# ziniuwan/maed

Hardware: AMD Instinct MI355X
Metric: video-clips/sec (BxT frames) train step (higher is better)
Workload: dtype bf16

## Files before the change

include/maed_hip.h:

```cpp
#ifndef MAED_HIP_H
#define MAED_HIP_H

#include <stddef.h>
#include <stdint.h>

#ifdef __cplusplus
extern "C" {
#endif

typedef enum { MAED_F32 = 0, MAED_BF16 = 1,
               MAED_F32X3 = 2, MAED_F32X6 = 3,
               MAED_F32X1 = 4 } maed_dtype;

typedef enum {
    MAED_OK = 0,
    MAED_ERR_ARG = -1,
    MAED_ERR_SHAPE = -2,
    MAED_ERR_ALIGN = -3,
    MAED_ERR_LAUNCH = -4,
    MAED_ERR_UNSUPPORTED = -5
} maed_status;

typedef enum {
    MAED_EPI_STORE = 0,
// ... 25 lines not shown
    MAED_OPT_ABLATE = 3,
    MAED_OPT_GN_BWD_ONEPASS = 4,
    MAED_OPT_F32_BWD_X1 = 5,
    MAED_OPT_ST_FUSED = 6,
    MAED_OPT_CONV3X3_ROWS_WGS = 7,
    MAED_OPT_STEM_WGRAD_WGS = 8,
    MAED_OPT_LBS_FRAMES = 9,
    MAED_OPT_TN_DMA = 10,
    MAED_OPT_X3_PLANES = 11,
    MAED_OPT_X3_PLANES_LN = 12,
    MAED_OPT_SK = 13,
    MAED_OPT_SK_GRID = 14,
    MAED_OPT_TN_SK = 15,
    MAED_OPT_CONV3X3_NARROW_WGS = 16,
    MAED_OPT_CONV3X3_FRAME = 17,
    MAED_OPT_COUNT
} maed_option;
int maed_init(int device);
int maed_device_faults(void);
int maed_device_faults_clear(void);
int maed_set_option(int key, int value);
int maed_get_option(int key);

int maed_layernorm_fwd(const float* x, int64_t x_row_stride, const float* gamma, const float* beta,
                       void* y, int dtype, float* mean, float* rstd,
                       int64_t rows, int C, float eps, void* stream);
int maed_layernorm_bwd(const void* dy, int dtype, const float* x, int64_t x_row_stride,
                       const float* gamma, const float* mean, const float* rstd,
                       const float* dres_in, float* dx_out, void* dx_twin, float* dgamma, float* dbeta,
                       int64_t rows, int C, void* stream);

int maed_gemm_nt(const void* A, int64_t lda, const void* B, int64_t ldb,
                 int64_t M, int64_t N, int64_t K, int dtype, int epilogue,
                 const float* bias, void* out, int64_t ldo, void* out2,
                 const void* aux, int64_t ldaux, int splitk, int impl, void* stream);

int maed_gemm_nt_planes(const void* a_hi, const void* a_lo, int64_t lda, const void* b_hi, const void* b_lo, int64_t ldb, int64_t M, int64_t N, int64_t K,
                        int epilogue, const float* bias, void* out, int64_t ldo, void* out2_bf16, const void* aux, int64_t ldaux, void* out_hi, void* out_lo,
                        int variant, void* stream);
int maed_split_planes(const float* x, void* hi, void* lo, int64_t n, void* stream);

int maed_gemm_tn_wgrad(const void* Y, int64_t ldy, const void* X, int64_t ldx, int64_t M, int N, int K,
                       float* dW, int64_t ldw, float* dbias, int dtype, void* stream);

int maed_transpose_cast(const void* in, int in_dtype, int64_t ldi, int64_t M, int64_t N,
                        void* out_t, int64_t ldt, void* out_c, int64_t ldc, float* colsum,
                        int dtype, void* stream);

int maed_attn_spatial_fwd(const void* qkv, void* o, float* lse, int F, int P, int H, float scale,
                          int dtype, int impl, void* stream);
int maed_attn_spatial_bwd(const void* qkv, const void* o, const void* d_o, const float* lse,
                          void* dqkv, int accumulate, int F, int P, int H, float scale,
                          int dtype, int impl, void* stream);

int maed_attn_temporal_fwd(const void* qkv, void* o, float* lse, int F, int P, int H, int T,
                           float scale, int dtype, void* stream);
int maed_attn_temporal_bwd(const void* qkv, const void* o, const void* d_o, const float* lse,
                           void* dqkv, int accumulate, int F, int P, int H, int T, float scale,
// ... 208 lines not shown
```

maed_amd/_lib.py:

```python
import ctypes as C
import os

HERE = os.path.dirname(os.path.abspath(__file__))
LIB_PATH = os.environ.get("MAED_HIP_LIB") or os.path.join(HERE, "libmaed_hip.so")

F32, BF16 = 0, 1
F32X3, F32X6, F32X1 = 2, 3, 4
EPI_STORE, EPI_GELU, EPI_RESID_F32, EPI_MUL_DGELU, EPI_ATOMIC_F32, EPI_STORE_F32, EPI_TANH, EPI_ADD = range(8)
IMPL_AUTO, IMPL_VALU, IMPL_MFMA = 0, 1, 2
IMPL_MFMA_256 = 6
IMPL_MFMA_LONG = 5
IMPL_MFMA_SK = 10
IMPL_X3, IMPL_X6, IMPL_X1 = 7, 8, 9
(OPT_F32_MATMUL, OPT_SIDE_STREAM, OPT_TN_TARGET_WGS, OPT_ABLATE, OPT_GN_BWD_ONEPASS, OPT_F32_BWD_X1, OPT_ST_FUSED, OPT_CONV3X3_ROWS_WGS, OPT_STEM_WGRAD_WGS,
 OPT_LBS_FRAMES, OPT_TN_DMA, OPT_X3_PLANES, OPT_X3_PLANES_LN, OPT_SK, OPT_SK_GRID, OPT_TN_SK, OPT_CONV3X3_NARROW_WGS, OPT_CONV3X3_FRAME) = range(18)

vp, i64, i32, f32 = C.c_void_p, C.c_int64, C.c_int, C.c_float


class GnAffineItem(C.Structure):
    _fields_ = [("ab", C.c_void_p), ("dgamma", C.c_void_p), ("dbeta", C.c_void_p), ("N", C.c_int), ("C", C.c_int)]


class BlockDims(C.Structure):
    _fields_ = [("F", i32), ("P", i32), ("C", i32), ("H", i32), ("T", i32), ("hidden", i32),
                ("dtype", i32), ("impl", i32), ("eps", f32)]


_PARAM_FIELDS = ["ln1_g", "ln1_b", "ln2_g", "ln2_b", "w_qkv", "w_ts", "w_proj", "w_fc1", "w_fc2",
                 "b_qkv", "b_ts", "b_proj", "b_fc1", "b_fc2", "wt_qkv", "wt_ts", "wt_proj", "wt_fc1", "wt_fc2"]
_GRAD_FIELDS = _PARAM_FIELDS[:14]


class BlockParams(C.Structure):
    _fields_ = [(n, vp) for n in _PARAM_FIELDS]

# ... 15 lines not shown


KTD_W_ANC = 3420

SIGNATURES = {
    "maed_last_error": (C.c_char_p, []),
    "maed_version": (i32, []),
    "maed_init": (i32, [i32]),
    "maed_device_faults": (i32, []),
    "maed_device_faults_clear": (i32, []),
    "maed_set_option": (i32, [i32, i32]),
    "maed_get_option": (i32, [i32]),
    "maed_layernorm_fwd": (i32, [vp, i64, vp, vp, vp, i32, vp, vp, i64, i32, f32, vp]),
    "maed_layernorm_bwd": (i32, [vp, i32, vp, i64, vp, vp, vp, vp, vp, vp, vp, vp, i64, i32, vp]),
    "maed_gemm_tn_wgrad": (i32, [vp, i64, vp, i64, i64, i32, i32, vp, i64, vp, i32, vp]),
    "maed_gemm_nt": (i32, [vp, i64, vp, i64, i64, i64, i64, i32, i32, vp, vp, i64, vp, vp, i64, i32, i32, vp]),
    "maed_transpose_cast": (i32, [vp, i32, i64, i64, i64, vp, i64, vp, i64, vp, i32, vp]),
    "maed_attn_spatial_fwd": (i32, [vp, vp, vp, i32, i32, i32, f32, i32, i32, vp]),
    "maed_attn_spatial_bwd": (i32, [vp, vp, vp, vp, vp, i32, i32, i32, i32, f32, i32, i32, vp]),
    "maed_attn_temporal_fwd": (i32, [vp, vp, vp, i32, i32, i32, i32, f32, i32, vp]),
    "maed_attn_temporal_bwd": (i32, [vp, vp, vp, vp, vp, i32, i32, i32, i32, i32, f32, i32, vp]),
    "maed_st_colmean": (i32, [vp, vp, vp, vp, i32, i32, i32, i32, vp]),
    "maed_st_mix_fwd": (i32, [vp, vp, vp, vp, i32, i32, i32, i32, vp]),
    "maed_st_mix_bwd_reduce": (i32, [vp, vp, vp, vp, vp, vp, i32, i32, i32, i32, vp]),
    "maed_st_mix_bwd_apply": (i32, [vp, vp, vp, vp, vp, i32, i32, i32, i32, vp]),
    "maed_st_fused_supported": (i32, [i32, i32, i32]),
    "maed_st_fused_fwd": (i32, [vp, vp, vp, vp, vp, vp, vp, vp, vp, i32, i32, i32, i32, vp]),
    "maed_st_fused_bwd": (i32, [vp, vp, vp, vp, vp, vp, vp, vp, vp, vp, i32, i32, i32, i32, vp]),
    "maed_embed_add_fwd": (i32, [vp, i32, vp, vp, vp, vp, i32, i32, i32, i32, vp]),
    "maed_embed_add_bwd": (i32, [vp, vp, i32, vp, vp, i32, i32, i32, i32, vp]),
# ... 109 lines not shown
    OPT_TN_TARGET_WGS: int(os.environ.get("MAED_TN_TARGET_WGS", "0")),
    OPT_ABLATE: int(os.environ.get("MAED_GEMM_ABLATE", "0")),
    OPT_F32_BWD_X1: int(os.environ.get("MAED_F32_BWD", "") == "bf16x1"),
    OPT_ST_FUSED: int(os.environ.get("MAED_ST_FUSED", "1")),
    OPT_GN_BWD_ONEPASS: int(os.environ.get("MAED_GN_BWD_ONEPASS", "1")),
    OPT_CONV3X3_ROWS_WGS: 0 if os.environ.get("MAED_CONV3X3_WGRAD_ROWS", "1") == "0" else int(os.environ.get("MAED_CONV3X3_ROWS_WGS", "256")),
    OPT_STEM_WGRAD_WGS: int(os.environ.get("MAED_STEM_WGS", "512")),
    OPT_LBS_FRAMES: int(os.environ.get("MAED_LBS_FB", "0")),
    OPT_TN_DMA: int(os.environ.get("MAED_TN_DMA", "1")),
    OPT_X3_PLANES: int(os.environ.get("MAED_X3_PLANES", "6")),
    OPT_SK: int(os.environ.get("MAED_SK", "1")),
    OPT_SK_GRID: int(os.environ.get("MAED_SK_GRID", "0")),
    OPT_CONV3X3_FRAME: int(os.environ.get("MAED_CONV3X3_FRAME", "1")),
    OPT_CONV3X3_NARROW_WGS: int(os.environ.get("MAED_CONV3X3_NARROW_WGS", "0")),
    OPT_TN_SK: int(os.environ.get("MAED_TN_SK", "1")),
    OPT_X3_PLANES_LN: int(os.environ.get("MAED_X3_PLANES_LN", "0")),
}


def apply_options(handle):
    for k, v in _OPTIONS.items():
        if handle.maed_set_option(k, v) != 0:
            raise MaedHipError(f"maed_set_option({k}, {v}) failed")


def set_option(key, value):
    _OPTIONS[key] = int(value)
    if _lib is not None:
        check(_lib.maed_set_option(key, int(value)), "set_option")

# ... 18 lines not shown
```

maed_amd/csrc/block.hip:

```cpp
#include "common.cuh"
#include "gemm_x3.h"
#include "prof.h"
#include <hip/hip_runtime.h>
#include <atomic>
#include <mutex>
#include <utility>
#include <vector>

static bool g_prof = false;
struct ProfRec { hipEvent_t a, b; double flops, bytes; };
static std::vector<ProfRec> g_prof_ev[PROF_NTAGS];
bool maed_prof_on() { return g_prof; }
void maed_prof_open(int tag, hipStream_t s, hipEvent_t* a) { (void)tag; (void)hipEventCreate(a); (void)hipEventRecord(*a, s); }
void maed_prof_close(int tag, hipStream_t s, hipEvent_t a, double flops, double bytes) {
    hipEvent_t b;
    (void)hipEventCreate(&b); (void)hipEventRecord(b, s);
    g_prof_ev[tag].push_back(ProfRec{a, b, flops, bytes});
}
extern "C" int maed_prof_enable(int on) { g_prof = on != 0; return MAED_OK; }
extern "C" int maed_prof_ntags(void) { return PROF_NTAGS; }
extern "C" int maed_prof_flops(double* flops) {
    for (int t = 0; t < PROF_NTAGS; ++t) {
        double tot = 0.0;
        for (auto& r : g_prof_ev[t]) tot += r.flops;
        if (flops) flops[t] = tot;
    }
    return MAED_OK;
}
extern "C" int maed_prof_records(int tag, double* us, double* flops, double* bytes, int cap) {
    if (tag < 0 || tag >= PROF_NTAGS) return 0;
    int i = 0;
    for (auto& r : g_prof_ev[tag]) {
        if (i < cap) {
            (void)hipEventSynchronize(r.b);
            float ms = 0.f;
            (void)hipEventElapsedTime(&ms, r.a, r.b);
            if (us) us[i] = 1e3 * (double)ms;
            if (flops) flops[i] = r.flops;
            if (bytes) bytes[i] = r.bytes;
        }
        ++i;
    }
    return i;
}
extern "C" int maed_prof_collect(double* ms_total, int* count) {
    for (int t = 0; t < PROF_NTAGS; ++t) {
        double tot = 0.0;
        for (auto& r : g_prof_ev[t]) {
            (void)hipEventSynchronize(r.b);
            float ms = 0.f;
            (void)hipEventElapsedTime(&ms, r.a, r.b);
            tot += ms;
            (void)hipEventDestroy(r.a); (void)hipEventDestroy(r.b);
        }
        if (ms_total) ms_total[t] = tot;
        if (count) count[t] = (int)g_prof_ev[t].size();
        g_prof_ev[t].clear();
    }
    return MAED_OK;
}
#define PROF(tag, expr) do { ProfScope ps__(tag, stream); MAED_PROPAGATE(expr); } while (0)

struct SideStream {
    hipStream_t s = nullptr;
    hipStream_t s2 = nullptr;
    hipEvent_t ev[64];
    hipEvent_t cast_ev[2];
    bool cast_pending[2] = {false, false};
    int next = 0;
    bool ok = false;
    void fence(hipStream_t from, hipStream_t to) {
// ... 331 lines not shown
    float* dxmid = (float*)(sc + S.dxmid);

    if (d->impl != MAED_IMPL_VALU && (dt == MAED_BF16 || (maed_x3_planes() && d->hidden % 4 == 0))) {
        const void* dyc = dt == MAED_F32 ? (const void*)dx_out : dx_out_twin;
        if (!dyc) {
            MAED_PROPAGATE(maed_transpose_cast(dx_out, MAED_F32, C, M, C, nullptr, 0, sc + S.dyc, C, nullptr, dt, stream));
            dyc = sc + S.dyc;
        }
        void* dxmid_tw = dt == MAED_F32 ? (void*)dxmid : (void*)(sc + S.dyt);
        SideStream* ss = side_stream();
        hipStream_t main_s = (hipStream_t)stream;
        void* wst = ss ? (void*)ss->s : stream;
#define TO_SIDE() do { if (ss) ss->fence(main_s, ss->s); } while (0)
#define FROM_SIDE() do { if (ss) ss->fence(ss->s, main_s); } while (0)
#define WGRAD(expr) do { ProfScope ps__(PROF_GEMM_WGRAD, wst); MAED_PROPAGATE(expr); } while (0)
        const int dmm = (dt == MAED_F32 && maed_opt(MAED_OPT_F32_BWD_X1)) ? MAED_F32X1 : dt;
        TO_SIDE();
        WGRAD(maed_gemm_tn_wgrad(dyc, C, sv + L.hact, Hd, M, C, Hd, g->w_fc2, Hd, g->b_fc2, dmm, wst));
        PROF(PROF_GEMM_DGRAD, maed_gemm_nt(dyc, C, p->wt_fc2, C, M, Hd, C, dmm, MAED_EPI_MUL_DGELU, nullptr, sc + S.bigA, Hd, nullptr, sv + L.hpre, Hd, 1, gi, stream));
        TO_SIDE();
        WGRAD(maed_gemm_tn_wgrad(sc + S.bigA, Hd, sv + L.ln2, C, M, Hd, C, g->w_fc1, C, g->b_fc1, dmm, wst));
        if (ss) MAED_HIP(hipEventRecord(ss->ev[63], ss->s), "ste_block_bwd: event");
        PROF(PROF_GEMM_DGRAD, maed_gemm_nt(sc + S.bigA, Hd, p->wt_fc1, Hd, M, C, Hd, dmm, MAED_EPI_STORE, nullptr, sc + S.act, C, nullptr, nullptr, 0, 1, gi, stream));
        const size_t big_t_bytes = (size_t)(Hd > 3 * C ? Hd : 3 * C) * (size_t)Mp * dtype_size(dt);
        const size_t ln_pb = (maed_layernorm_bwd_partials_bytes(M, C) + 255) & ~(size_t)255;
        float* ln_part = 2 * ln_pb <= big_t_bytes ? (float*)(sc + S.bigT) : nullptr;
        float* ln_part1 = ln_part ? (float*)(sc + S.bigT + ln_pb) : nullptr;
        const bool ln_side = ss != nullptr && ln_part != nullptr && maed_opt(MAED_OPT_ST_FUSED) == 4;
        const bool piggy = st_fused(*d) && maed_opt(MAED_OPT_ST_FUSED) != 2 && (int64_t)d->F * 16 <= 256 * ((M + 31) / 32);
        MAED_PROPAGATE(maed_layernorm_bwd_ws(sc + S.act, dt, (const float*)(sv + L.xmid), C, p->ln2_g, (const float*)(sv + L.mean2), (const float*)(sv + L.rstd2),
                                             dx_out, dxmid, dt == MAED_F32 ? nullptr : dxmid_tw, g->ln2_g, g->ln2_b, M, C, ln_part, stream, !ln_side,
                                             piggy ? (uint32_t*)(sv + L.st_sync) : nullptr, piggy ? d->F * 16 : 0));
        if (ln_side) { TO_SIDE(); MAED_PROPAGATE(maed_layernorm_affine_finish(ln_part, M, C, g->ln2_g, g->ln2_b, wst)); }
        TO_SIDE();
        WGRAD(maed_gemm_tn_wgrad(dxmid_tw, C, sv + L.mix, C, M, C, C, g->w_proj, C, g->b_proj, dmm, wst));
        PROF(PROF_GEMM_DGRAD, maed_gemm_nt(dxmid_tw, C, p->wt_proj, C, M, C, C, dmm, MAED_EPI_STORE, nullptr, sc + S.act, C, nullptr, nullptr, 0, 1, gi, stream));
        if (st_fused(*d)) {
            PROF(PROF_ST_BWD, maed_st_fused_bwd_ws(sc + S.act, sv + L.xs, sv + L.xt, logits, p->wt_ts, sc + S.dlog, sc + S.dxs, sc + S.dxt, (uint32_t*)(sv + L.st_sync),
                                                   (float*)(sv + L.st_ex), d->F, d->P, C, dt, !piggy, 0u, stream));
            TO_SIDE();
            WGRAD(maed_gemm_tn_wgrad(sc + S.dlog, 2 * C, sv + L.means, 2 * C, d->F, 2 * C, 2 * C, g->w_ts, 2 * C, g->b_ts, dmm, wst));
        } else {
            MAED_PROPAGATE(maed_st_mix_bwd_reduce(sc + S.act, sv + L.xs, sv + L.xt, logits, sc + S.dlog, (float*)(sc + S.ws), d->F, d->P, C, dt, stream));
            TO_SIDE();
            WGRAD(maed_gemm_tn_wgrad(sc + S.dlog, 2 * C, sv + L.means, 2 * C, d->F, 2 * C, 2 * C, g->w_ts, 2 * C, g->b_ts, dmm, wst));
            MAED_PROPAGATE(maed_gemm_nt(sc + S.dlog, 2 * C, p->wt_ts, 2 * C, d->F, 2 * C, 2 * C, dmm, MAED_EPI_STORE, nullptr, sc + S.dmeans, 2 * C, nullptr, nullptr, 0, 1, gi, stream));
            MAED_PROPAGATE(maed_st_mix_bwd_apply(sc + S.act, logits, sc + S.dmeans, sc + S.dxs, sc + S.dxt, d->F, d->P, C, dt, stream));
        }
        if (ss) MAED_HIP(hipStreamWaitEvent(main_s, ss->ev[63], 0), "ste_block_bwd: stream wait");
        PROF(PROF_ATTN_TM_BWD, maed_attn_temporal_bwd(sv + L.qkv, sv + L.xt, sc + S.dxt, (const float*)(sv + L.lse_t), sc + S.bigA, 0, d->F, d->P, d->H, d->T, scale, dt, stream));
        PROF(PROF_ATTN_SP_BWD, maed_attn_spatial_bwd(sv + L.qkv, sv + L.xs, sc + S.dxs, (const float*)(sv + L.lse_s), sc + S.bigA, 1, d->F, d->P, d->H, scale, dt,
                                                     MAED_IMPL_AUTO, stream));
        TO_SIDE();
        WGRAD(maed_gemm_tn_wgrad(sc + S.bigA, 3 * C, sv + L.ln1, C, M, 3 * C, C, g->w_qkv, C, g->b_qkv, dmm, wst));
        PROF(PROF_GEMM_DGRAD, maed_gemm_nt(sc + S.bigA, 3 * C, p->wt_qkv, 3 * C, M, C, 3 * C, dmm, MAED_EPI_STORE, nullptr, sc + S.act, C, nullptr, nullptr, 0, 1, gi, stream));
        MAED_PROPAGATE(maed_layernorm_bwd_ws(sc + S.act, dt, x_in, C, p->ln1_g, (const float*)(sv + L.mean1), (const float*)(sv + L.rstd1), dxmid, dx_in,
                                             dx_in_twin, g->ln1_g, g->ln1_b, M, C, ln_part1, stream, !ln_side));
        if (ln_side) { TO_SIDE(); MAED_PROPAGATE(maed_layernorm_affine_finish(ln_part1, M, C, g->ln1_g, g->ln1_b, wst)); }
        FROM_SIDE();
#undef TO_SIDE
#undef FROM_SIDE
#undef WGRAD
        return MAED_OK;
    }
    MAED_PROPAGATE(maed_transpose_cast(dx_out, MAED_F32, C, M, C, sc + S.dyt, Mp, sc + S.dyc, C, g->b_fc2, dt, stream));
    MAED_PROPAGATE(maed_transpose_cast(sv + L.hact, dt, Hd, M, Hd, sc + S.bigT, Mp, nullptr, 0, nullptr, dt, stream));
    PROF(PROF_GEMM_WGRAD, wgrad(sc + S.dyt, sc + S.bigT, C, Hd, Mp, g->w_fc2, *d, stream));
    MAED_PROPAGATE(maed_gemm_nt(sc + S.dyc, C, p->wt_fc2, C, M, Hd, C, dt, MAED_EPI_MUL_DGELU, nullptr, sc + S.bigA, Hd, nullptr, sv + L.hpre, Hd, 1, gi, stream));
    MAED_PROPAGATE(maed_transpose_cast(sc + S.bigA, dt, Hd, M, Hd, sc + S.bigT, Mp, nullptr, 0, g->b_fc1, dt, stream));
    MAED_PROPAGATE(maed_transpose_cast(sv + L.ln2, dt, C, M, C, sc + S.xT, Mp, nullptr, 0, nullptr, dt, stream));
    PROF(PROF_GEMM_WGRAD, wgrad(sc + S.bigT, sc + S.xT, Hd, C, Mp, g->w_fc1, *d, stream));
    MAED_PROPAGATE(maed_gemm_nt(sc + S.bigA, Hd, p->wt_fc1, Hd, M, C, Hd, dt, MAED_EPI_STORE, nullptr, sc + S.act, C, nullptr, nullptr, 0, 1, gi, stream));
    MAED_PROPAGATE(maed_layernorm_bwd(sc + S.act, dt, (const float*)(sv + L.xmid), C, p->ln2_g, (const float*)(sv + L.mean2), (const float*)(sv + L.rstd2),
                                      dx_out, dxmid, nullptr, g->ln2_g, g->ln2_b, M, C, stream));
    MAED_PROPAGATE(maed_transpose_cast(dxmid, MAED_F32, C, M, C, sc + S.dyt, Mp, sc + S.dyc, C, g->b_proj, dt, stream));
    MAED_PROPAGATE(maed_transpose_cast(sv + L.mix, dt, C, M, C, sc + S.xT, Mp, nullptr, 0, nullptr, dt, stream));
    PROF(PROF_GEMM_WGRAD, wgrad(sc + S.dyt, sc + S.xT, C, C, Mp, g->w_proj, *d, stream));
// ... 33 lines not shown
```

maed_amd/csrc/gemm_tn.hip:

```cpp
#include "common.cuh"
#include "gemm_epilogue.cuh"
#include "gemm_x3.h"
#include "prof.h"
#include <stdlib.h>

int maed_tn_splits(int tiles) {
    const int target = maed_opt(MAED_OPT_TN_TARGET_WGS);
    if (target > 0) return (target + tiles - 1) / tiles;
    if (tiles >= 32) return 512 / tiles > 0 ? 512 / tiles : 1;
    return (256 + tiles - 1) / tiles;
}
static int tn_remap() { return 1; }

bool maed_gemm_tn_sk_ok(int64_t M, int N, int K, int64_t ldy, int64_t ldx, int64_t ldw, const void* Y, const void* X, const void* dW);
int maed_gemm_tn_sk_launch(const void* Y, int64_t ldy, const void* X, int64_t ldx, int64_t M, int N, int K, float* dW, int64_t ldw, float* dbias, int grid_opt, hipStream_t s);
int maed_sk_cus(void);
bool maed_gemm_tn_dma_ok(int64_t M, int N, int K, int64_t ldy, int64_t ldx);
int maed_gemm_tn_dma_launch(const void* Y, int64_t ldy, const void* X, int64_t ldx, int64_t M, int N, int K, float* dW, int64_t ldw, float* dbias, int which, hipStream_t stream);
bool maed_conv3x3_wgrad_rows64_ok(int F, int H, int W, int Cin, int Cout);
int maed_conv3x3_wgrad_rows64_launch(const void* dy, const void* x, float* dW, void* scratch, int F, int H, int W, hipStream_t stream);

#define TN_BM 64
#define TN_LD 72

__device__ __forceinline__ uint32_t perm_lo(uint32_t a, uint32_t b) { return __builtin_amdgcn_perm(b, a, 0x05040100u); }
__device__ __forceinline__ uint32_t perm_hi(uint32_t a, uint32_t b) { return __builtin_amdgcn_perm(b, a, 0x07060302u); }

struct TnConv { const uint16_t* tapmask; const bf16* zero_page; int Cin, Wimg;
                const int* rowtab = nullptr; };

template <bool CONV, bool S2 = false>
__global__ __launch_bounds__(256, 2) void gemm_tn_mfma_bf16_kernel(const bf16* __restrict__ Y, int64_t ldy, const bf16* __restrict__ X,
                                                                   int64_t ldx, int64_t M, int N, int K, float* __restrict__ dW,
// ... 189 lines not shown
    if (splits > (nmt + 3) / 4) splits = (nmt + 3) / 4;
    if (splits < 1) splits = 1;
    const int per = (nmt + splits - 1) / splits;
    const int z = (nmt + per - 1) / per;
#ifdef MAED_GEMM_ABLATE
    hipLaunchKernelGGL(gemm_tn_mfma_bf16_kernel<false>, dim3(tn * tk, 1, z), dim3(256), 0, (hipStream_t)stream, (const bf16*)Y, ldy, (const bf16*)X, ldx, M,
                       N, K, dW, ldw, dbias, tk, per, TnConv{nullptr, nullptr, 0, 0}, tn_remap(), maed_opt(MAED_OPT_ABLATE));
#else
    hipLaunchKernelGGL(gemm_tn_mfma_bf16_kernel<false>, dim3(tn * tk, 1, z), dim3(256), 0, (hipStream_t)stream, (const bf16*)Y, ldy, (const bf16*)X, ldx, M,
                       N, K, dW, ldw, dbias, tk, per, TnConv{nullptr, nullptr, 0, 0}, tn_remap());
#endif
    MAED_CHECK_LAUNCH("gemm_tn_wgrad");
    return MAED_OK;
}

__global__ __launch_bounds__(256) void conv_tapmask_kernel(uint16_t* __restrict__ mask, int64_t M, int64_t Mpad, int H, int W) {
    const int64_t m = (int64_t)blockIdx.x * 256 + threadIdx.x;
    if (m >= Mpad) return;
    unsigned bits = 0;
    if (m < M) {
        const int x = (int)(m % W), y = (int)((m / W) % H);
#pragma unroll
        for (int t = 0; t < 9; ++t) {
            const int yy = y + t / 3 - 1, xx = x + t % 3 - 1;
            bits |= ((unsigned)yy < (unsigned)H && (unsigned)xx < (unsigned)W ? 1u : 0u) << t;
        }
    }
    mask[m] = (uint16_t)bits;
}

// ... 110 lines not shown
```

maed_amd/csrc/gemm_tn2.hip:

```cpp
#include "common.cuh"
#include "gemm_epilogue.cuh"
#include "prof.h"

#define T2_BM 32
#define T2_STAGES 4

template <int NWR, int NWC, int RN, int RK>
__global__ __launch_bounds__(NWR * NWC * 64, (NWR * NWC) / 4) void gemm_tn_dma_bf16_kernel(const bf16* __restrict__ Y, int64_t ldy, const bf16* __restrict__ X, int64_t ldx,
                                                                                             int64_t M, int N, int K, float* __restrict__ dW, int64_t ldw,
                                                                                             float* __restrict__ dbias, int tiles_k, int mtiles_per_split, int remap) {
    constexpr int NW = NWR * NWC, TN = NWR * RN * 32, TK = NWC * RK * 32;
    constexpr int STAGE_ELEMS = T2_BM * (TN + TK);
    constexpr int NINSTR = STAGE_ELEMS / 512, IPW = NINSTR / NW;
    constexpr int YINSTR = T2_BM * TN / 512;
    static_assert(NINSTR % NW == 0 && TN % 128 == 0 && TK % 128 == 0, "tile / wave layout");
    MAED_DYN_SHARED(unsigned short, lds);
    const int tid = threadIdx.x, lane = tid & 63, wave = __builtin_amdgcn_readfirstlane(tid >> 6);
    const int wr = wave / NWC, wc = wave % NWC, l31 = lane & 31, hi = lane >> 5, i16 = lane & 15;
    const int lin = remap ? xcd_remap((int)(blockIdx.z * gridDim.x + blockIdx.x), (int)(gridDim.x * gridDim.z)) : (int)(blockIdx.z * gridDim.x + blockIdx.x);
    const int bx = lin % (int)gridDim.x, bz = lin / (int)gridDim.x;
    const int tile_n = bx / tiles_k, tile_k = bx % tiles_k;
    const int n0 = tile_n * TN, k0 = tile_k * TK;
    const int nmt = (int)(M / T2_BM);
    const int mt_beg = bz * mtiles_per_split;
    int mt_end = mt_beg + mtiles_per_split;
    if (mt_end > nmt) mt_end = nmt;
    if (mt_beg >= mt_end) return;
    const int nt = mt_end - mt_beg;

    uint32_t voff[IPW];
    const char* sbase[IPW]; int64_t sld[IPW];
#pragma unroll
    for (int i = 0; i < IPW; ++i) {
        const int q = wave * IPW + i, side = q >= YINSTR;
        const int cols = side ? TK : TN, cpr = cols / 8;
// ... 70 lines not shown
#pragma unroll
            for (int r = 0; r < 16; ++r) {
                const int nrow = n0 + (wr * RN + a) * 32 + (r & 3) + 8 * (r >> 2) + 4 * hi;
                if (nrow < N && kcol < K) atomicAdd(dW + (int64_t)nrow * ldw + kcol, acc[a][b][r]);
            }
        }
    if (bias_blk && l31 == 0) {
#pragma unroll
        for (int a = 0; a < RN; ++a)
#pragma unroll
            for (int r = 0; r < 16; ++r) {
                const int n = n0 + (wr * RN + a) * 32 + (r & 3) + 8 * (r >> 2) + 4 * hi;
                if (n < N) atomicAdd(dbias + n, accb[a][r]);
            }
    }
}

bool maed_gemm_tn_dma_ok(int64_t M, int N, int K, int64_t ldy, int64_t ldx) {
    return M >= T2_BM && M % T2_BM == 0 && N % 8 == 0 && K % 8 == 0 && ldy % 8 == 0 && ldx % 8 == 0 && ldy < (1 << 24) && ldx < (1 << 24)
           && (int64_t)T2_BM * (ldy > ldx ? ldy : ldx) * 2 + 1024 < (1ll << 31);
}

int maed_tn_splits(int tiles);

int maed_gemm_tn_dma_launch(const void* Y, int64_t ldy, const void* X, int64_t ldx, int64_t M, int N, int K, float* dW, int64_t ldw, float* dbias, int which,
                            hipStream_t stream) {
    const bool big = which == 3;
    const int T = big ? 256 : 128;
    const int tn = (N + T - 1) / T, tk = (K + T - 1) / T;
    const int nmt = (int)(M / T2_BM);
// ... 7 lines not shown
    if (big) {
        constexpr size_t lds = (size_t)T2_STAGES * T2_BM * 512 * 2;
        static bool attr_set = false;
        if (!attr_set) { (void)hipFuncSetAttribute((const void*)gemm_tn_dma_bf16_kernel<2, 4, 4, 2>, hipFuncAttributeMaxDynamicSharedMemorySize, (int)lds); attr_set = true; }
        hipLaunchKernelGGL((gemm_tn_dma_bf16_kernel<2, 4, 4, 2>), dim3(tn * tk, 1, z), dim3(512), lds, stream, (const bf16*)Y, ldy, (const bf16*)X, ldx, M, N, K, dW, ldw, dbias,
                           tk, per, 1);
    } else {
        constexpr size_t lds = (size_t)T2_STAGES * T2_BM * 256 * 2;
        static bool attr_set = false;
        if (!attr_set) { (void)hipFuncSetAttribute((const void*)gemm_tn_dma_bf16_kernel<2, 2, 2, 2>, hipFuncAttributeMaxDynamicSharedMemorySize, (int)lds); attr_set = true; }
        hipLaunchKernelGGL((gemm_tn_dma_bf16_kernel<2, 2, 2, 2>), dim3(tn * tk, 1, z), dim3(256), lds, stream, (const bf16*)Y, ldy, (const bf16*)X, ldx, M, N, K, dW, ldw, dbias,
                           tk, per, 1);
    }
    return MAED_OK;
}
```

maed_amd/csrc/gemm_tn_sk.hip:

```cpp
#include "common.cuh"
#include "gemm_epilogue.cuh"
#include <mutex>

#define TS_T 256
#define TS_BK 64
#define TS_SLOT (TS_BK * 128)
#define TS_A0 0
#define TS_B0 1
#define TS_B1 2
#define TS_A1 3
#define TS_RING_ELEMS (2 * 4 * TS_SLOT)
#define TS_LDS_ELEMS (TS_RING_ELEMS + 4 * 2048)
#define TS_STAGE_BYTE0 (7 * TS_SLOT * 2)
#define TS_SLAB_FLOATS (TS_T * TS_T + TS_T)
#define TS_UNI(x_) ((uint32_t)__builtin_amdgcn_readfirstlane((int)(x_)))
#ifdef MAED_HOSTSIM
#define TS_OPAQUE(v_) ((void)0)
#else
#define TS_OPAQUE(v_) asm volatile("" : "+v"(v_))
#endif

__device__ __forceinline__ float ts_sum8(const bf16x8_t& f, float acc) {
    uint4 u;
    __builtin_memcpy(&u, &f, 16);
// ... 218 lines not shown
        const int nn = n0 + (int)threadIdx.x;
        float b = 0.f;
#pragma unroll 8
        for (int g = g0; g < g1; ++g) b += slabs[(int64_t)g * TS_SLAB_FLOATS + TS_T * TS_T + threadIdx.x];
        if (nn < N) dbias[nn] += b;
    }
}

float* maed_sk_slab_set(hipStream_t s, size_t* bytes, int* ncu);

bool maed_gemm_tn_sk_ok(int64_t M, int N, int K, int64_t ldy, int64_t ldx, int64_t ldw, const void* Y, const void* X, const void* dW) {
    return M >= 128 && M % 128 == 0 && N >= 256 && K >= 256 && N % 8 == 0 && K % 8 == 0 && ldy % 8 == 0 && ldx % 8 == 0 && ldw % 4 == 0
           && (M * (ldy > ldx ? ldy : ldx) * 2) < (1ll << 40) && (int64_t)TS_BK * (ldy > ldx ? ldy : ldx) * 2 + 65536 < (1ll << 31)
           && is_aligned(Y, 16) && is_aligned(X, 16) && is_aligned(dW, 16);
}
int maed_gemm_tn_sk_launch(const void* Y, int64_t ldy, const void* X, int64_t ldx, int64_t M, int N, int K, float* dW, int64_t ldw, float* dbias, int grid_opt,
                           hipStream_t s) {
    size_t bytes = 0;
    int ncu = 0;
    float* slabs = maed_sk_slab_set(s, &bytes, &ncu);
    if (!slabs) return MAED_ERR_UNSUPPORTED;
    TsPlan P;
    const int tn = (N + TS_T - 1) / TS_T, tk = (K + TS_T - 1) / TS_T;
    P.tiles = tn * tk; P.tiles_k = tk; P.pairs = (int)(M / 128);
    int G = grid_opt > 0 && grid_opt < ncu ? grid_opt : ncu;
    if ((size_t)G * TS_SLAB_FLOATS * sizeof(float) > bytes) G = (int)(bytes / (TS_SLAB_FLOATS * sizeof(float)));
    if (P.tiles > G || P.pairs < 1) return MAED_ERR_UNSUPPORTED;
    if (grid_opt <= 0 && (int64_t)P.tiles * P.pairs < (int64_t)32 * G) return MAED_ERR_UNSUPPORTED;
    if (dbias) hipLaunchKernelGGL(gemm_tn_sk_bf16_kernel<true>, dim3((unsigned)G), dim3(512), 0, s, (const bf16*)Y, ldy, (const bf16*)X, ldx, N, K, P, slabs);
    else hipLaunchKernelGGL(gemm_tn_sk_bf16_kernel<false>, dim3((unsigned)G), dim3(512), 0, s, (const bf16*)Y, ldy, (const bf16*)X, ldx, N, K, P, slabs);
    hipLaunchKernelGGL(gemm_tn_sk_reduce_kernel, dim3(TS_T / 4, (unsigned)P.tiles), dim3(256), 0, s, (const float*)slabs, dW, ldw, dbias, N, K, P, G);
    return MAED_OK;
}
```

maed_amd/csrc/options.hip:

```cpp
#include "common.cuh"
#include "gemm_x3.h"
#include <atomic>
#include <string.h>

static std::atomic<int> g_opt[MAED_OPT_COUNT] = {
    {0},
    {1},
    {0},
    {0},
    {1},
    {0},
    {1},
    {256},
    {512},
    {0},
    {1},
    {6},
    {0},
    {1},
    {0},
    {1},
    {0},
    {1},
};

extern "C" int maed_init(int device) {
#ifndef MAED_HOSTSIM
    hipDeviceProp_t prop;
    if (hipGetDeviceProperties(&prop, device) != hipSuccess) { (void)hipGetLastError(); maed_set_error("init: no HIP device %d", device); return MAED_ERR_ARG; }
    if (!strstr(prop.gcnArchName, "gfx950")) {
        maed_set_error("init: device %d is %s; libmaed_hip is built for gfx950 (MI355X) only", device, prop.gcnArchName);
        return MAED_ERR_UNSUPPORTED;
    }
#else
    (void)device;
#endif
    (void)maed_fault_word();
// ... 42 lines not shown
                       "NaN-poisoned, the one-pass GroupNorm backward and the fused attentive addition run as their multi-launch forms from the next call on", n);
    return n;
}
extern "C" int maed_device_faults_clear(void) { uint32_t* w = g_fault.load(std::memory_order_acquire); if (w) *(volatile uint32_t*)w = 0; g_fault_told.store(0); return MAED_OK; }

extern "C" int maed_set_option(int key, int value) {
    MAED_CHECK_ARG(key >= 0 && key < MAED_OPT_COUNT, MAED_ERR_ARG, "set_option: unknown option %d", key);
    if (key == MAED_OPT_F32_MATMUL) MAED_CHECK_ARG(value >= 0 && value <= 2, MAED_ERR_ARG, "set_option: MAED_OPT_F32_MATMUL takes 0 (exact), 1 (bf16x3) or 2 (bf16x6)");
    if (key == MAED_OPT_TN_TARGET_WGS) MAED_CHECK_ARG(value == 0 || value >= 64, MAED_ERR_ARG, "set_option: MAED_OPT_TN_TARGET_WGS must be 0 (heuristic) or >= 64");
    if (key == MAED_OPT_CONV3X3_ROWS_WGS || key == MAED_OPT_STEM_WGRAD_WGS) MAED_CHECK_ARG(value >= 0 && value <= 65535, MAED_ERR_ARG, "set_option: workgroup count out of range");
    if (key == MAED_OPT_LBS_FRAMES) MAED_CHECK_ARG(value == 0 || value == 4 || value == 8 || value == 16, MAED_ERR_ARG, "set_option: MAED_OPT_LBS_FRAMES takes 0 (auto), 4, 8 or 16");
    if (key == MAED_OPT_X3_PLANES) MAED_CHECK_ARG(value == 0 || (value >= 2 && value <= 7 && value != 3), MAED_ERR_ARG, "set_option: MAED_OPT_X3_PLANES takes 0 (fp32 operands) or a kernel variant 2, 4, 5, 6, 7");
    if (key == MAED_OPT_SK) MAED_CHECK_ARG(value >= 0 && value <= 3, MAED_ERR_ARG, "set_option: MAED_OPT_SK takes 0 (off), 1 (heuristic), 2 (no K cuts) or 3 (always)");
    if (key == MAED_OPT_TN_SK) MAED_CHECK_ARG(value == 0 || value == 1, MAED_ERR_ARG, "set_option: MAED_OPT_TN_SK takes 0 or 1");
    if (key == MAED_OPT_SK_GRID) MAED_CHECK_ARG(value >= 0 && value <= 512, MAED_ERR_ARG, "set_option: MAED_OPT_SK_GRID takes 0 (one workgroup per CU) or a workgroup count <= 512");
    g_opt[key].store(value, std::memory_order_relaxed);
    return MAED_OK;
}

extern "C" int maed_get_option(int key) {
    if (key < 0 || key >= MAED_OPT_COUNT) { maed_set_error("get_option: unknown option %d", key); return MAED_ERR_ARG; }
    return g_opt[key].load(std::memory_order_relaxed);
}

int maed_opt(int key) { return g_opt[key].load(std::memory_order_relaxed); }

int maed_x3_planes(void) {
    const int v = maed_opt(MAED_OPT_F32_MATMUL);
    return v == 1 ? 2 : v == 2 ? 3 : 0;
}
// ... 1 lines not shown
```

maed_amd/csrc/prof.h:

```cpp
#pragma once
#include "common.cuh"

enum { PROF_ATTN_SP_FWD = 0, PROF_ATTN_TM_FWD, PROF_GEMM_QKV, PROF_GEMM_FC1, PROF_GEMM_FC2, PROF_ATTN_SP_BWD, PROF_ATTN_TM_BWD, PROF_GEMM_WGRAD,
       PROF_GEMM_PROJ, PROF_GEMM_DGRAD , PROF_LAYERNORM ,
       PROF_TN_ALL , PROF_TN_CONV ,
       PROF_ST_FWD, PROF_ST_BWD , PROF_NTAGS };

bool maed_prof_on();
void maed_prof_open(int tag, hipStream_t s, hipEvent_t* a);
void maed_prof_close(int tag, hipStream_t s, hipEvent_t a, double flops, double bytes);

struct ProfScope {
    int tag; hipStream_t s; hipEvent_t a; bool on; double flops, bytes;
    ProfScope(int tag_, void* stream, double flops_ = 0.0, double bytes_ = 0.0)
        : tag(tag_), s((hipStream_t)stream), a(nullptr), on(maed_prof_on()), flops(flops_), bytes(bytes_) {
        if (on) maed_prof_open(tag, s, &a);
    }
    ~ProfScope() { if (on) maed_prof_close(tag, s, a, flops, bytes); }
};
```

Measured before the change: 419.3.

## Group weight-gradient GEMMs into a single multi-problem DMA kernel launch

```diff
diff --git a/include/maed_hip.h b/include/maed_hip.h
--- a/include/maed_hip.h
+++ b/include/maed_hip.h
@@ -63,6 +63,7 @@
     MAED_OPT_TN_SK = 15,
     MAED_OPT_CONV3X3_NARROW_WGS = 16,
     MAED_OPT_CONV3X3_FRAME = 17,
+    MAED_OPT_TN_GROUP = 18,
     MAED_OPT_COUNT
 } maed_option;
 int maed_init(int device);
@@ -91,6 +92,16 @@
 
 int maed_gemm_tn_wgrad(const void* Y, int64_t ldy, const void* X, int64_t ldx, int64_t M, int N, int K,
                        float* dW, int64_t ldw, float* dbias, int dtype, void* stream);
+
+#define MAED_TN_GROUP_MAX 8
+typedef struct {
+    const void* Y; int64_t ldy;
+    const void* X; int64_t ldx;
+    int N, K;
+    float* dW; int64_t ldw;
+    float* dbias;
+} maed_tn_problem;
+int maed_gemm_tn_wgrad_grouped(const maed_tn_problem* problems, int n, int64_t M, int dtype, void* stream);
 
 int maed_transpose_cast(const void* in, int in_dtype, int64_t ldi, int64_t M, int64_t N,
                         void* out_t, int64_t ldt, void* out_c, int64_t ldc, float* colsum,
diff --git a/maed_amd/_lib.py b/maed_amd/_lib.py
--- a/maed_amd/_lib.py
+++ b/maed_amd/_lib.py
@@ -13,13 +13,18 @@
 IMPL_MFMA_SK = 10
 IMPL_X3, IMPL_X6, IMPL_X1 = 7, 8, 9
 (OPT_F32_MATMUL, OPT_SIDE_STREAM, OPT_TN_TARGET_WGS, OPT_ABLATE, OPT_GN_BWD_ONEPASS, OPT_F32_BWD_X1, OPT_ST_FUSED, OPT_CONV3X3_ROWS_WGS, OPT_STEM_WGRAD_WGS,
- OPT_LBS_FRAMES, OPT_TN_DMA, OPT_X3_PLANES, OPT_X3_PLANES_LN, OPT_SK, OPT_SK_GRID, OPT_TN_SK, OPT_CONV3X3_NARROW_WGS, OPT_CONV3X3_FRAME) = range(18)
+ OPT_LBS_FRAMES, OPT_TN_DMA, OPT_X3_PLANES, OPT_X3_PLANES_LN, OPT_SK, OPT_SK_GRID, OPT_TN_SK, OPT_CONV3X3_NARROW_WGS, OPT_CONV3X3_FRAME, OPT_TN_GROUP) = range(19)
 
 vp, i64, i32, f32 = C.c_void_p, C.c_int64, C.c_int, C.c_float
 
 
 class GnAffineItem(C.Structure):
     _fields_ = [("ab", C.c_void_p), ("dgamma", C.c_void_p), ("dbeta", C.c_void_p), ("N", C.c_int), ("C", C.c_int)]
+
+
+class TnProblem(C.Structure):
+    _fields_ = [("Y", C.c_void_p), ("ldy", C.c_int64), ("X", C.c_void_p), ("ldx", C.c_int64), ("N", C.c_int), ("K", C.c_int),
+                ("dW", C.c_void_p), ("ldw", C.c_int64), ("dbias", C.c_void_p)]
 
 
 class BlockDims(C.Structure):
@@ -65,6 +70,7 @@
     "maed_layernorm_fwd": (i32, [vp, i64, vp, vp, vp, i32, vp, vp, i64, i32, f32, vp]),
     "maed_layernorm_bwd": (i32, [vp, i32, vp, i64, vp, vp, vp, vp, vp, vp, vp, vp, i64, i32, vp]),
     "maed_gemm_tn_wgrad": (i32, [vp, i64, vp, i64, i64, i32, i32, vp, i64, vp, i32, vp]),
+    "maed_gemm_tn_wgrad_grouped": (i32, [C.POINTER(TnProblem), i32, i64, i32, vp]),
     "maed_gemm_nt": (i32, [vp, i64, vp, i64, i64, i64, i64, i32, i32, vp, vp, i64, vp, vp, i64, i32, i32, vp]),
     "maed_transpose_cast": (i32, [vp, i32, i64, i64, i64, vp, i64, vp, i64, vp, i32, vp]),
     "maed_attn_spatial_fwd": (i32, [vp, vp, vp, i32, i32, i32, f32, i32, i32, vp]),
@@ -204,6 +210,7 @@
     OPT_CONV3X3_FRAME: int(os.environ.get("MAED_CONV3X3_FRAME", "1")),
     OPT_CONV3X3_NARROW_WGS: int(os.environ.get("MAED_CONV3X3_NARROW_WGS", "0")),
     OPT_TN_SK: int(os.environ.get("MAED_TN_SK", "1")),
+    OPT_TN_GROUP: int(os.environ.get("MAED_TN_GROUP", "1")),
     OPT_X3_PLANES_LN: int(os.environ.get("MAED_X3_PLANES_LN", "0")),
 }
 
diff --git a/maed_amd/csrc/block.hip b/maed_amd/csrc/block.hip
--- a/maed_amd/csrc/block.hip
+++ b/maed_amd/csrc/block.hip
@@ -8,14 +8,14 @@
 #include <vector>
 
 static bool g_prof = false;
-struct ProfRec { hipEvent_t a, b; double flops, bytes; };
+struct ProfRec { hipEvent_t a, b; double flops, bytes; int launches; };
 static std::vector<ProfRec> g_prof_ev[PROF_NTAGS];
 bool maed_prof_on() { return g_prof; }
 void maed_prof_open(int tag, hipStream_t s, hipEvent_t* a) { (void)tag; (void)hipEventCreate(a); (void)hipEventRecord(*a, s); }
-void maed_prof_close(int tag, hipStream_t s, hipEvent_t a, double flops, double bytes) {
+void maed_prof_close(int tag, hipStream_t s, hipEvent_t a, double flops, double bytes, int launches) {
     hipEvent_t b;
     (void)hipEventCreate(&b); (void)hipEventRecord(b, s);
-    g_prof_ev[tag].push_back(ProfRec{a, b, flops, bytes});
+    g_prof_ev[tag].push_back(ProfRec{a, b, flops, bytes, launches});
 }
 extern "C" int maed_prof_enable(int on) { g_prof = on != 0; return MAED_OK; }
 extern "C" int maed_prof_ntags(void) { return PROF_NTAGS; }
@@ -46,15 +46,17 @@
 extern "C" int maed_prof_collect(double* ms_total, int* count) {
     for (int t = 0; t < PROF_NTAGS; ++t) {
         double tot = 0.0;
+        int launches = 0;
         for (auto& r : g_prof_ev[t]) {
             (void)hipEventSynchronize(r.b);
             float ms = 0.f;
             (void)hipEventElapsedTime(&ms, r.a, r.b);
             tot += ms;
+            launches += r.launches;
             (void)hipEventDestroy(r.a); (void)hipEventDestroy(r.b);
         }
         if (ms_total) ms_total[t] = tot;
-        if (count) count[t] = (int)g_prof_ev[t].size();
+        if (count) count[t] = launches;
         g_prof_ev[t].clear();
     }
     return MAED_OK;
@@ -416,12 +418,22 @@
 #define TO_SIDE() do { if (ss) ss->fence(main_s, ss->s); } while (0)
 #define FROM_SIDE() do { if (ss) ss->fence(ss->s, main_s); } while (0)
 #define WGRAD(expr) do { ProfScope ps__(PROF_GEMM_WGRAD, wst); MAED_PROPAGATE(expr); } while (0)
+#define WGRAD2(expr) do { ProfScope ps__(PROF_GEMM_WGRAD, wst, 0.0, 0.0, 2); MAED_PROPAGATE(expr); } while (0)
         const int dmm = (dt == MAED_F32 && maed_opt(MAED_OPT_F32_BWD_X1)) ? MAED_F32X1 : dt;
-        TO_SIDE();
-        WGRAD(maed_gemm_tn_wgrad(dyc, C, sv + L.hact, Hd, M, C, Hd, g->w_fc2, Hd, g->b_fc2, dmm, wst));
+        const int tng = dmm == MAED_BF16 ? maed_opt(MAED_OPT_TN_GROUP) : 0;
+        const bool group_a = tng != 0, group_b = tng == 1;
+        if (!group_a) {
+            TO_SIDE();
+            WGRAD(maed_gemm_tn_wgrad(dyc, C, sv + L.hact, Hd, M, C, Hd, g->w_fc2, Hd, g->b_fc2, dmm, wst));
+        }
         PROF(PROF_GEMM_DGRAD, maed_gemm_nt(dyc, C, p->wt_fc2, C, M, Hd, C, dmm, MAED_EPI_MUL_DGELU, nullptr, sc + S.bigA, Hd, nullptr, sv + L.hpre, Hd, 1, gi, stream));
         TO_SIDE();
-        WGRAD(maed_gemm_tn_wgrad(sc + S.bigA, Hd, sv + L.ln2, C, M, Hd, C, g->w_fc1, C, g->b_fc1, dmm, wst));
+        if (group_a) {
+            const maed_tn_problem pa[2] = {{dyc, C, sv + L.hact, Hd, C, Hd, g->w_fc2, Hd, g->b_fc2}, {sc + S.bigA, Hd, sv + L.ln2, C, Hd, C, g->w_fc1, C, g->b_fc1}};
+            WGRAD2(maed_gemm_tn_wgrad_grouped(pa, 2, M, dmm, wst));
+        } else {
+            WGRAD(maed_gemm_tn_wgrad(sc + S.bigA, Hd, sv + L.ln2, C, M, Hd, C, g->w_fc1, C, g->b_fc1, dmm, wst));
+        }
         if (ss) MAED_HIP(hipEventRecord(ss->ev[63], ss->s), "ste_block_bwd: event");
         PROF(PROF_GEMM_DGRAD, maed_gemm_nt(sc + S.bigA, Hd, p->wt_fc1, Hd, M, C, Hd, dmm, MAED_EPI_STORE, nullptr, sc + S.act, C, nullptr, nullptr, 0, 1, gi, stream));
         const size_t big_t_bytes = (size_t)(Hd > 3 * C ? Hd : 3 * C) * (size_t)Mp * dtype_size(dt);
@@ -434,8 +446,10 @@
                                              dx_out, dxmid, dt == MAED_F32 ? nullptr : dxmid_tw, g->ln2_g, g->ln2_b, M, C, ln_part, stream, !ln_side,
                                              piggy ? (uint32_t*)(sv + L.st_sync) : nullptr, piggy ? d->F * 16 : 0));
         if (ln_side) { TO_SIDE(); MAED_PROPAGATE(maed_layernorm_affine_finish(ln_part, M, C, g->ln2_g, g->ln2_b, wst)); }
-        TO_SIDE();
-        WGRAD(maed_gemm_tn_wgrad(dxmid_tw, C, sv + L.mix, C, M, C, C, g->w_proj, C, g->b_proj, dmm, wst));
+        if (!group_b) {
+            TO_SIDE();
+            WGRAD(maed_gemm_tn_wgrad(dxmid_tw, C, sv + L.mix, C, M, C, C, g->w_proj, C, g->b_proj, dmm, wst));
+        }
         PROF(PROF_GEMM_DGRAD, maed_gemm_nt(dxmid_tw, C, p->wt_proj, C, M, C, C, dmm, MAED_EPI_STORE, nullptr, sc + S.act, C, nullptr, nullptr, 0, 1, gi, stream));
         if (st_fused(*d)) {
             PROF(PROF_ST_BWD, maed_st_fused_bwd_ws(sc + S.act, sv + L.xs, sv + L.xt, logits, p->wt_ts, sc + S.dlog, sc + S.dxs, sc + S.dxt, (uint32_t*)(sv + L.st_sync),
@@ -454,7 +468,12 @@
         PROF(PROF_ATTN_SP_BWD, maed_attn_spatial_bwd(sv + L.qkv, sv + L.xs, sc + S.dxs, (const float*)(sv + L.lse_s), sc + S.bigA, 1, d->F, d->P, d->H, scale, dt,
                                                      MAED_IMPL_AUTO, stream));
         TO_SIDE();
-        WGRAD(maed_gemm_tn_wgrad(sc + S.bigA, 3 * C, sv + L.ln1, C, M, 3 * C, C, g->w_qkv, C, g->b_qkv, dmm, wst));
+        if (group_b) {
+            const maed_tn_problem pb[2] = {{dxmid_tw, C, sv + L.mix, C, C, C, g->w_proj, C, g->b_proj}, {sc + S.bigA, 3 * C, sv + L.ln1, C, 3 * C, C, g->w_qkv, C, g->b_qkv}};
+            WGRAD2(maed_gemm_tn_wgrad_grouped(pb, 2, M, dmm, wst));
+        } else {
+            WGRAD(maed_gemm_tn_wgrad(sc + S.bigA, 3 * C, sv + L.ln1, C, M, 3 * C, C, g->w_qkv, C, g->b_qkv, dmm, wst));
+        }
         PROF(PROF_GEMM_DGRAD, maed_gemm_nt(sc + S.bigA, 3 * C, p->wt_qkv, 3 * C, M, C, 3 * C, dmm, MAED_EPI_STORE, nullptr, sc + S.act, C, nullptr, nullptr, 0, 1, gi, stream));
         MAED_PROPAGATE(maed_layernorm_bwd_ws(sc + S.act, dt, x_in, C, p->ln1_g, (const float*)(sv + L.mean1), (const float*)(sv + L.rstd1), dxmid, dx_in,
                                              dx_in_twin, g->ln1_g, g->ln1_b, M, C, ln_part1, stream, !ln_side));
@@ -463,6 +482,7 @@
 #undef TO_SIDE
 #undef FROM_SIDE
 #undef WGRAD
+#undef WGRAD2
         return MAED_OK;
     }
     MAED_PROPAGATE(maed_transpose_cast(dx_out, MAED_F32, C, M, C, sc + S.dyt, Mp, sc + S.dyc, C, g->b_fc2, dt, stream));
diff --git a/maed_amd/csrc/gemm_tn.hip b/maed_amd/csrc/gemm_tn.hip
--- a/maed_amd/csrc/gemm_tn.hip
+++ b/maed_amd/csrc/gemm_tn.hip
@@ -14,9 +14,11 @@
 
 bool maed_gemm_tn_sk_ok(int64_t M, int N, int K, int64_t ldy, int64_t ldx, int64_t ldw, const void* Y, const void* X, const void* dW);
 int maed_gemm_tn_sk_launch(const void* Y, int64_t ldy, const void* X, int64_t ldx, int64_t M, int N, int K, float* dW, int64_t ldw, float* dbias, int grid_opt, hipStream_t s);
+bool maed_gemm_tn_sk_pays(int64_t M, int N, int K, int grid_opt, int G);
 int maed_sk_cus(void);
 bool maed_gemm_tn_dma_ok(int64_t M, int N, int K, int64_t ldy, int64_t ldx);
 int maed_gemm_tn_dma_launch(const void* Y, int64_t ldy, const void* X, int64_t ldx, int64_t M, int N, int K, float* dW, int64_t ldw, float* dbias, int which, hipStream_t stream);
+int maed_gemm_tn_dma_group_launch(const maed_tn_problem* pr, int n, int64_t M, hipStream_t stream);
 bool maed_conv3x3_wgrad_rows64_ok(int F, int H, int W, int Cin, int Cout);
 int maed_conv3x3_wgrad_rows64_launch(const void* dy, const void* x, float* dW, void* scratch, int F, int H, int W, hipStream_t stream);
 
@@ -236,6 +238,34 @@
     return MAED_OK;
 }
 
+extern "C" int maed_gemm_tn_wgrad_grouped(const maed_tn_problem* pr, int n, int64_t M, int dtype, void* stream) {
+    MAED_CHECK_ARG(pr && n >= 1 && n <= MAED_TN_GROUP_MAX, MAED_ERR_ARG, "gemm_tn_wgrad_grouped: need 1 .. %d problems (n=%d)", MAED_TN_GROUP_MAX, n);
+    const int tnd = maed_opt(MAED_OPT_TN_DMA);
+    bool grouped = n >= 2 && dtype == MAED_BF16 && maed_opt(MAED_OPT_TN_GROUP) != 0 && (tnd == 1 || tnd == 2 || tnd == 4) && M > 0;
+    double flops = 0.0, bytes = 0.0;
+    for (int i = 0; grouped && i < n; ++i) {
+        const maed_tn_problem& q = pr[i];
+        grouped = q.Y && q.X && q.dW && q.N > 0 && q.K > 0 && q.ldy >= q.N && q.ldx >= q.K && q.ldw >= q.K && is_aligned(q.Y, 16) && is_aligned(q.X, 16)
+                  && maed_gemm_tn_dma_ok(M, q.N, q.K, q.ldy, q.ldx) && !(tnd == 4 && M >= 65536 && (int64_t)q.N * q.K <= 65536);
+        if (grouped && maed_opt(MAED_OPT_TN_SK) && maed_gemm_tn_sk_ok(M, q.N, q.K, q.ldy, q.ldx, q.ldw, q.Y, q.X, q.dW)
+            && ((q.N + 255) / 256) * ((q.K + 255) / 256) * 2 <= maed_sk_cus()) {
+            const int ncu = maed_sk_cus(), go = maed_opt(MAED_OPT_SK_GRID);
+            if (maed_gemm_tn_sk_pays(M, q.N, q.K, go, go > 0 && go < ncu ? go : ncu)) grouped = false;
+        }
+        flops += 2.0 * (double)M * q.N * q.K;
+        bytes += 2.0 * (double)M * ((double)q.N + q.K) + 4.0 * (double)q.N * q.K;
+    }
+    if (!grouped) {
+        for (int i = 0; i < n; ++i)
+            MAED_PROPAGATE(maed_gemm_tn_wgrad(pr[i].Y, pr[i].ldy, pr[i].X, pr[i].ldx, M, pr[i].N, pr[i].K, pr[i].dW, pr[i].ldw, pr[i].dbias, dtype, stream));
+        return MAED_OK;
+    }
+    ProfScope prof__(PROF_TN_ALL, stream, flops, bytes);
+    MAED_PROPAGATE(maed_gemm_tn_dma_group_launch(pr, n, M, (hipStream_t)stream));
+    MAED_CHECK_LAUNCH("gemm_tn_wgrad_grouped");
+    return MAED_OK;
+}
+
 __global__ __launch_bounds__(256) void conv_tapmask_kernel(uint16_t* __restrict__ mask, int64_t M, int64_t Mpad, int H, int W) {
     const int64_t m = (int64_t)blockIdx.x * 256 + threadIdx.x;
     if (m >= Mpad) return;
diff --git a/maed_amd/csrc/gemm_tn2.hip b/maed_amd/csrc/gemm_tn2.hip
--- a/maed_amd/csrc/gemm_tn2.hip
+++ b/maed_amd/csrc/gemm_tn2.hip
@@ -1,14 +1,14 @@
 #include "common.cuh"
 #include "gemm_epilogue.cuh"
 #include "prof.h"
+#include <limits.h>
 
 #define T2_BM 32
 #define T2_STAGES 4
 
 template <int NWR, int NWC, int RN, int RK>
-__global__ __launch_bounds__(NWR * NWC * 64, (NWR * NWC) / 4) void gemm_tn_dma_bf16_kernel(const bf16* __restrict__ Y, int64_t ldy, const bf16* __restrict__ X, int64_t ldx,
-                                                                                             int64_t M, int N, int K, float* __restrict__ dW, int64_t ldw,
-                                                                                             float* __restrict__ dbias, int tiles_k, int mtiles_per_split, int remap) {
+__device__ __forceinline__ void tn_dma_tile(const bf16* __restrict__ Y, int64_t ldy, const bf16* __restrict__ X, int64_t ldx, int64_t M, int N, int K,
+                                            float* __restrict__ dW, int64_t ldw, float* __restrict__ dbias, int tiles_k, int mtiles_per_split, int bx, int bz) {
     constexpr int NW = NWR * NWC, TN = NWR * RN * 32, TK = NWC * RK * 32;
     constexpr int STAGE_ELEMS = T2_BM * (TN + TK);
     constexpr int NINSTR = STAGE_ELEMS / 512, IPW = NINSTR / NW;
@@ -17,8 +17,6 @@
     MAED_DYN_SHARED(unsigned short, lds);
     const int tid = threadIdx.x, lane = tid & 63, wave = __builtin_amdgcn_readfirstlane(tid >> 6);
     const int wr = wave / NWC, wc = wave % NWC, l31 = lane & 31, hi = lane >> 5, i16 = lane & 15;
-    const int lin = remap ? xcd_remap((int)(blockIdx.z * gridDim.x + blockIdx.x), (int)(gridDim.x * gridDim.z)) : (int)(blockIdx.z * gridDim.x + blockIdx.x);
-    const int bx = lin % (int)gridDim.x, bz = lin / (int)gridDim.x;
     const int tile_n = bx / tiles_k, tile_k = bx % tiles_k;
     const int n0 = tile_n * TN, k0 = tile_k * TK;
     const int nmt = (int)(M / T2_BM);
@@ -119,6 +117,29 @@
                 if (n < N) atomicAdd(dbias + n, accb[a][r]);
             }
     }
+}
+
+template <int NWR, int NWC, int RN, int RK>
+__global__ __launch_bounds__(NWR * NWC * 64, (NWR * NWC) / 4) void gemm_tn_dma_bf16_kernel(const bf16* __restrict__ Y, int64_t ldy, const bf16* __restrict__ X, int64_t ldx,
+                                                                                             int64_t M, int N, int K, float* __restrict__ dW, int64_t ldw,
+                                                                                             float* __restrict__ dbias, int tiles_k, int mtiles_per_split, int remap) {
+    const int lin = remap ? xcd_remap((int)(blockIdx.z * gridDim.x + blockIdx.x), (int)(gridDim.x * gridDim.z)) : (int)(blockIdx.z * gridDim.x + blockIdx.x);
+    const int bx = lin % (int)gridDim.x, bz = lin / (int)gridDim.x;
+    tn_dma_tile<NWR, NWC, RN, RK>(Y, ldy, X, ldx, M, N, K, dW, ldw, dbias, tiles_k, mtiles_per_split, bx, bz);
+}
+
+struct TnGroupMember { const bf16* Y; const bf16* X; float* dW; float* dbias; int64_t ldy, ldx, ldw; int N, K, tiles_k, tile_beg; };
+struct TnGroupArgs { TnGroupMember m[MAED_TN_GROUP_MAX]; };
+
+__global__ __launch_bounds__(256, 1) void gemm_tn_dma_group_bf16_kernel(TnGroupArgs g, int64_t M, int mtiles_per_split) {
+    const int lin = xcd_remap((int)(blockIdx.z * gridDim.x + blockIdx.x), (int)(gridDim.x * gridDim.z));
+    const int bx = lin % (int)gridDim.x, bz = lin / (int)gridDim.x;
+    int p = 0;
+#pragma unroll
+    for (int i = 1; i < MAED_TN_GROUP_MAX; ++i) p = bx >= g.m[i].tile_beg ? i : p;
+    p = __builtin_amdgcn_readfirstlane(p);
+    const TnGroupMember& m = g.m[p];
+    tn_dma_tile<2, 2, 2, 2>(m.Y, m.ldy, m.X, m.ldx, M, m.N, m.K, m.dW, m.ldw, m.dbias, m.tiles_k, mtiles_per_split, bx - m.tile_beg, bz);
 }
 
 bool maed_gemm_tn_dma_ok(int64_t M, int N, int K, int64_t ldy, int64_t ldx) {
@@ -156,3 +177,26 @@
     }
     return MAED_OK;
 }
+
+int maed_gemm_tn_dma_group_launch(const maed_tn_problem* pr, int n, int64_t M, hipStream_t stream) {
+    TnGroupArgs g;
+    int tiles = 0;
+    for (int i = 0; i < MAED_TN_GROUP_MAX; ++i) {
+        TnGroupMember& m = g.m[i];
+        if (i >= n) { m = TnGroupMember{nullptr, nullptr, nullptr, nullptr, 0, 0, 0, 0, 0, 1, INT_MAX}; continue; }
+        const int tn = (pr[i].N + 127) / 128, tk = (pr[i].K + 127) / 128;
+        m = TnGroupMember{(const bf16*)pr[i].Y, (const bf16*)pr[i].X, pr[i].dW, pr[i].dbias, pr[i].ldy, pr[i].ldx, pr[i].ldw, pr[i].N, pr[i].K, tk, tiles};
+        tiles += tn * tk;
+    }
+    const int nmt = (int)(M / T2_BM);
+    int splits = 512 / tiles;
+    if (splits > (nmt + 7) / 8) splits = (nmt + 7) / 8;
+    if (splits < 1) splits = 1;
+    const int per = (nmt + splits - 1) / splits;
+    const int z = (nmt + per - 1) / per;
+    constexpr size_t lds = (size_t)T2_STAGES * T2_BM * 256 * 2;
+    static bool attr_set = false;
+    if (!attr_set) { (void)hipFuncSetAttribute((const void*)gemm_tn_dma_group_bf16_kernel, hipFuncAttributeMaxDynamicSharedMemorySize, (int)lds); attr_set = true; }
+    hipLaunchKernelGGL(gemm_tn_dma_group_bf16_kernel, dim3(tiles, 1, z), dim3(256), lds, stream, g, M, per);
+    return MAED_OK;
+}
diff --git a/maed_amd/csrc/gemm_tn_sk.hip b/maed_amd/csrc/gemm_tn_sk.hip
--- a/maed_amd/csrc/gemm_tn_sk.hip
+++ b/maed_amd/csrc/gemm_tn_sk.hip
@@ -256,6 +256,10 @@
            && (M * (ldy > ldx ? ldy : ldx) * 2) < (1ll << 40) && (int64_t)TS_BK * (ldy > ldx ? ldy : ldx) * 2 + 65536 < (1ll << 31)
            && is_aligned(Y, 16) && is_aligned(X, 16) && is_aligned(dW, 16);
 }
+bool maed_gemm_tn_sk_pays(int64_t M, int N, int K, int grid_opt, int G) {
+    const int64_t tiles = (int64_t)((N + TS_T - 1) / TS_T) * ((K + TS_T - 1) / TS_T), pairs = M / 128;
+    return tiles <= G && pairs >= 1 && (grid_opt > 0 || tiles * pairs >= (int64_t)32 * G);
+}
 int maed_gemm_tn_sk_launch(const void* Y, int64_t ldy, const void* X, int64_t ldx, int64_t M, int N, int K, float* dW, int64_t ldw, float* dbias, int grid_opt,
                            hipStream_t s) {
     size_t bytes = 0;
@@ -267,8 +271,7 @@
     P.tiles = tn * tk; P.tiles_k = tk; P.pairs = (int)(M / 128);
     int G = grid_opt > 0 && grid_opt < ncu ? grid_opt : ncu;
     if ((size_t)G * TS_SLAB_FLOATS * sizeof(float) > bytes) G = (int)(bytes / (TS_SLAB_FLOATS * sizeof(float)));
-    if (P.tiles > G || P.pairs < 1) return MAED_ERR_UNSUPPORTED;
-    if (grid_opt <= 0 && (int64_t)P.tiles * P.pairs < (int64_t)32 * G) return MAED_ERR_UNSUPPORTED;
+    if (!maed_gemm_tn_sk_pays(M, N, K, grid_opt, G)) return MAED_ERR_UNSUPPORTED;
     if (dbias) hipLaunchKernelGGL(gemm_tn_sk_bf16_kernel<true>, dim3((unsigned)G), dim3(512), 0, s, (const bf16*)Y, ldy, (const bf16*)X, ldx, N, K, P, slabs);
     else hipLaunchKernelGGL(gemm_tn_sk_bf16_kernel<false>, dim3((unsigned)G), dim3(512), 0, s, (const bf16*)Y, ldy, (const bf16*)X, ldx, N, K, P, slabs);
     hipLaunchKernelGGL(gemm_tn_sk_reduce_kernel, dim3(TS_T / 4, (unsigned)P.tiles), dim3(256), 0, s, (const float*)slabs, dW, ldw, dbias, N, K, P, G);
diff --git a/maed_amd/csrc/options.hip b/maed_amd/csrc/options.hip
--- a/maed_amd/csrc/options.hip
+++ b/maed_amd/csrc/options.hip
@@ -21,6 +21,7 @@
     {0},
     {1},
     {0},
+    {1},
     {1},
 };
 
@@ -93,6 +94,7 @@
     if (key == MAED_OPT_SK) MAED_CHECK_ARG(value >= 0 && value <= 3, MAED_ERR_ARG, "set_option: MAED_OPT_SK takes 0 (off), 1 (heuristic), 2 (no K cuts) or 3 (always)");
     if (key == MAED_OPT_TN_SK) MAED_CHECK_ARG(value == 0 || value == 1, MAED_ERR_ARG, "set_option: MAED_OPT_TN_SK takes 0 or 1");
     if (key == MAED_OPT_SK_GRID) MAED_CHECK_ARG(value >= 0 && value <= 512, MAED_ERR_ARG, "set_option: MAED_OPT_SK_GRID takes 0 (one workgroup per CU) or a workgroup count <= 512");
+    if (key == MAED_OPT_TN_GROUP) MAED_CHECK_ARG(value >= 0 && value <= 2, MAED_ERR_ARG, "set_option: MAED_OPT_TN_GROUP takes 0 (member by member), 1 (grouped) or 2 (fc2 + fc1 only)");
     g_opt[key].store(value, std::memory_order_relaxed);
     return MAED_OK;
 }
diff --git a/maed_amd/csrc/prof.h b/maed_amd/csrc/prof.h
--- a/maed_amd/csrc/prof.h
+++ b/maed_amd/csrc/prof.h
@@ -8,13 +8,14 @@
 
 bool maed_prof_on();
 void maed_prof_open(int tag, hipStream_t s, hipEvent_t* a);
-void maed_prof_close(int tag, hipStream_t s, hipEvent_t a, double flops, double bytes);
+void maed_prof_close(int tag, hipStream_t s, hipEvent_t a, double flops, double bytes, int launches = 1);
 
 struct ProfScope {
     int tag; hipStream_t s; hipEvent_t a; bool on; double flops, bytes;
-    ProfScope(int tag_, void* stream, double flops_ = 0.0, double bytes_ = 0.0)
-        : tag(tag_), s((hipStream_t)stream), a(nullptr), on(maed_prof_on()), flops(flops_), bytes(bytes_) {
+    int launches;
+    ProfScope(int tag_, void* stream, double flops_ = 0.0, double bytes_ = 0.0, int launches_ = 1)
+        : tag(tag_), s((hipStream_t)stream), a(nullptr), on(maed_prof_on()), flops(flops_), bytes(bytes_), launches(launches_) {
         if (on) maed_prof_open(tag, s, &a);
     }
-    ~ProfScope() { if (on) maed_prof_close(tag, s, a, flops, bytes); }
+    ~ProfScope() { if (on) maed_prof_close(tag, s, a, flops, bytes, launches); }
 };
```

Result: no change. 416.1 (-0.8%).
